# NikolayKrivosheev/Distributed-deep-learning-on-personal-computers

Measured on AMD Instinct MI355X. Metric: images/sec (whole node), U-Net 256x256 6-class tiles, higher is better.
Workload: dtype bf16

## Files before the change

csrc/bindings.cpp:

```cpp
#include <ATen/ATen.h>
#include <c10/core/DeviceGuard.h>
#include <c10/hip/HIPStream.h>
#include <torch/library.h>

#include <cstdlib>
#include <mutex>
#include <string>
#include <unordered_map>
#include <vector>

#include "ops.h"

namespace ddlpc {

namespace {

hipStream_t cur_stream() { return c10::hip::getCurrentHIPStream().stream(); }

#define CHECK_DEV(t) TORCH_CHECK((t).is_cuda(), #t " must be a GPU tensor")
#define CHECK_CONTIG(t) TORCH_CHECK((t).is_contiguous(), #t " must be contiguous")
#define CHECK_BF16(t) TORCH_CHECK((t).scalar_type() == at::kBFloat16, #t " must be bf16")
#define CHECK_F32(t) TORCH_CHECK((t).scalar_type() == at::kFloat, #t " must be fp32")

const bf16_t* bptr(const at::Tensor& t) { return reinterpret_cast<const bf16_t*>(t.data_ptr()); }
// ... 28 lines not shown
    TD = 1;
    TW = W >= 16 ? 16 : 8;
    TH = BM / TW;
  } else {
    TW = W >= 16 ? 16 : 8;
    TH = 4;
    TD = BM / (TW * TH);
  }
}

int pick_bn(int Cout) {
  if (Cout <= 32) return 32;
  if (Cout <= 64) return 64;
  return 128;
}

}

namespace {
thread_local std::string g_last_path;
}
void set_last_path(const std::string& path) { g_last_path = path; }
std::string last_path() { return g_last_path; }

namespace {
const char* const kKnobs[] = {"CROP_LDS_T"};
bool knob_registered(const std::string& name) {
  for (const char* k : kKnobs)
    if (k[0] != 0 && name == k) return true;
  return false;
}
std::mutex g_knob_mu;
std::unordered_map<std::string, int>& knob_map() {
  static std::unordered_map<std::string, int> m;
  return m;
}
}

int knob(const char* name, int def) {
  TORCH_CHECK(knob_registered(name), "knob '", name, "' read but not listed in kKnobs");
  std::lock_guard<std::mutex> lk(g_knob_mu);
  auto& m = knob_map();
  auto it = m.find(name);
  if (it != m.end()) return it->second;
  const std::string env = std::string("DDLPC_") + name;
  const char* e = getenv(env.c_str());
  const int v = e ? atoi(e) : def;
  m.emplace(name, v);
  return v;
// ... 970 lines not shown
                                    const at::Tensor& labels, const at::Tensor& out3,
                                    const c10::optional<at::Tensor>& gscale, int64_t ignore_index,
                                    const c10::optional<at::Tensor>& dw_out,
                                    const c10::optional<at::Tensor>& db_out,
                                    const c10::optional<at::Tensor>& bn4, bool store_da) {
  CHECK_DEV(a); CHECK_CONTIG(a);
  c10::DeviceGuard guard(a.device());
  const int C = (int)a.size(-1), K = (int)Wh.size(0);
  const float* pbn = bn4_ptr(bn4, C);
  TORCH_CHECK(head_supported(C, K), "head kernel: unsupported (C, K)");
  TORCH_CHECK(store_da || pbn != nullptr, "head_ce_bwd: store_da=False needs the deferred BN (bn4)");
  const long long P = a.numel() / C;
  const int nb = head_ce_bwd_blocks(C, K, pbn != nullptr, P, num_cus());
  auto fopts = a.options().dtype(at::kFloat);
  at::Tensor dA = store_da ? at::empty_like(a) : at::empty({0}, a.options());
  at::Tensor part = at::empty({nb, K * C + K}, fopts);
  at::Tensor bnpart = pbn != nullptr ? at::empty({nb, 2, C}, fopts) : at::empty({0}, fopts);
  head_ce_bwd_launch(bptr(a), Wh.data_ptr<float>(), bh.data_ptr<float>(), labels.data_ptr<int64_t>(),
                     fptr_opt(gscale), out3.data_ptr<float>(), 0, store_da ? bptr_mut(dA) : nullptr,
                     part.data_ptr<float>(), nb, P, C, K, (int)ignore_index, pbn,
                     pbn != nullptr ? bnpart.data_ptr<float>() : nullptr, cur_stream());
  set_last_path(std::string("head_ce_bwd:") + head_variant(C) + (pbn != nullptr ? ":defer" : "") +
                (store_da ? "" : ":stats"));
  const bool into = dw_out.has_value() && dw_out->defined();
  at::Tensor sums = reduce_rows(part, nb, K * C + K);
  if (into) {
    TORCH_CHECK(dw_out->is_contiguous() && db_out->is_contiguous(), "grad outs must be contiguous");
    scatter_sums_launch(sums.data_ptr<double>(), K * C, dw_out->data_ptr<float>(), 2, 0, 0, 0, 1.f,
                        true, cur_stream());
    scatter_sums_launch(sums.data_ptr<double>() + K * C, K, db_out->data_ptr<float>(), 2, 0, 0, 0,
                        1.f, true, cur_stream());
    at::Tensor none = at::empty({0}, fopts);
    return {dA, none, none, bnpart};
  }
  at::Tensor red = at::empty({K * C + K}, fopts);
  scatter_sums_launch(sums.data_ptr<double>(), K * C + K, red.data_ptr<float>(), 2, 0, 0, 0, 1.f,
                      false, cur_stream());
  at::Tensor dW = red.narrow(0, 0, K * C).view({K, C});
  at::Tensor db = red.narrow(0, K * C, K);
  return {dA, dW, db, bnpart};
}

std::vector<at::Tensor> head_ce_bn_bwd(const at::Tensor& a, const at::Tensor& Wh, const at::Tensor& bh,
                                       const at::Tensor& labels, const at::Tensor& out3,
                                       const c10::optional<at::Tensor>& gscale, int64_t ignore_index,
                                       const at::Tensor& bn4, const at::Tensor& partial,
// ... 9 lines not shown
    const long long P = a.numel() / C;
    TORCH_CHECK(C == 32 && K <= 16 && P % (groups * 16) == 0,
                "head_ce_bn_bwd groups: C = 32 head, pixels per group a multiple of 16");
    CHECK_F32(bn4); CHECK_CONTIG(bn4); CHECK_F32(partial); CHECK_CONTIG(partial); CHECK_F32(gamma);
    TORCH_CHECK(bn4.numel() == groups * 4 * C && partial.numel() % (groups * 2 * C) == 0,
                "head_ce_bn_bwd groups: bn4 [groups][4][C], partial [groups * R][2][C]");
    auto fopts = a.options().dtype(at::kFloat);
    const bool into = dgamma_out.has_value() && dgamma_out->defined();
    at::Tensor dgamma = into ? *dgamma_out : at::empty({C}, fopts);
    at::Tensor dbeta = into ? *dbeta_out : at::empty({C}, fopts);
    at::Tensor coefs = at::empty({groups, 3, C}, fopts);
    at::Tensor gsum = at::empty({groups, 2, C}, a.options().dtype(at::kDouble));
    const int nb = (int)(partial.numel() / (groups * 2 * C));
    bn_group_grad_rows_launch(partial.data_ptr<float>(), nb, (int)groups, C, (double)(P / groups),
                              gamma.data_ptr<float>(), bn4.data_ptr<float>(), dgamma.data_ptr<float>(),
                              dbeta.data_ptr<float>(), into, coefs.data_ptr<float>(),
                              gsum.data_ptr<double>(), ps, cur_stream());
    at::Tensor dY = at::empty_like(a);
    head_bn_apply_launch(bptr(a), Wh.data_ptr<float>(), bh.data_ptr<float>(), labels.data_ptr<int64_t>(),
                         fptr_opt(gscale), out3.data_ptr<float>(), bn4.data_ptr<float>(),
                         coefs.data_ptr<float>(), bptr_mut(dY), P, C, K, (int)ignore_index, num_cus(),
                         cur_stream(), (int)groups);
    set_last_path("head_ce_bn_bwd:head32:groups");
    return {dY, dgamma, dbeta};
  }
  const float* pbn = bn4_ptr(bn4, C);
  TORCH_CHECK(head_supported(C, K), "head kernel: unsupported (C, K)");
  CHECK_F32(partial); CHECK_CONTIG(partial); CHECK_F32(gamma);
  TORCH_CHECK(partial.numel() % (2 * C) == 0 && partial.numel() > 0, "partial rows must be [R][2][C]");
  const long long P = a.numel() / C;
  const int nb = (int)(partial.numel() / (2 * C));
  auto fopts = a.options().dtype(at::kFloat);
  const bool into = dgamma_out.has_value() && dgamma_out->defined();
  at::Tensor dgamma = into ? *dgamma_out : at::empty({C}, fopts);
  at::Tensor dbeta = into ? *dbeta_out : at::empty({C}, fopts);
  at::Tensor coefs = at::empty({3, C}, fopts);
  const float* s = pbn;
  if (nb <= 2048) {
    bn_grad_finalize_rows_launch(partial.data_ptr<float>(), nb, C, (double)P, gamma.data_ptr<float>(),
                                 s + C, dgamma.data_ptr<float>(), dbeta.data_ptr<float>(),
                                 coefs.data_ptr<float>(), into, cur_stream(), ps);
  } else {
    at::Tensor sums = reduce_rows(partial, nb, 2 * C);
    bn_grad_finalize_launch(sums.data_ptr<double>(), C, (double)P, gamma.data_ptr<float>(), s + C,
                            dgamma.data_ptr<float>(), dbeta.data_ptr<float>(),
                            coefs.data_ptr<float>(), into, cur_stream(), ps);
  }
  at::Tensor dY = at::empty_like(a);
  head_bn_apply_launch(bptr(a), Wh.data_ptr<float>(), bh.data_ptr<float>(), labels.data_ptr<int64_t>(),
                       fptr_opt(gscale), out3.data_ptr<float>(), pbn, coefs.data_ptr<float>(),
                       bptr_mut(dY), P, C, K, (int)ignore_index, num_cus(), cur_stream());
  set_last_path(std::string("head_ce_bn_bwd:") + head_variant(C));
  return {dY, dgamma, dbeta};
}

std::vector<at::Tensor> head_ce_fwd_stats(const at::Tensor& a, const at::Tensor& Wh,
                                          const at::Tensor& bh, const at::Tensor& labels,
                                          int64_t ignore_index, const at::Tensor& bn4,
                                          int64_t groups) {
  CHECK_DEV(a); CHECK_CONTIG(a); CHECK_BF16(a); CHECK_CONTIG(labels);
  TORCH_CHECK(labels.scalar_type() == at::kLong, "labels must be int64");
  c10::DeviceGuard guard(a.device());
  const int C = (int)a.size(-1), K = (int)Wh.size(0);
  const long long P = a.numel() / C;
  const float* pbn = nullptr;
  if (groups > 1) {
    CHECK_F32(bn4); CHECK_CONTIG(bn4);
    TORCH_CHECK(C == 32 && K <= 16 && P % (groups * 16) == 0 && bn4.numel() == groups * 4 * C,
                "head_ce_fwd_stats groups: C = 32 head, bn4 [groups][4][C], pixels per group a "
                "multiple of 16");
    pbn = bn4.data_ptr<float>();
  } else {
    pbn = bn4_ptr(bn4, C);
  }
  TORCH_CHECK(head_supported(C, K), "head kernel: unsupported (C, K)");
  TORCH_CHECK(labels.numel() == P, "labels / activation pixel count mismatch");
  const int nb = head_fwd_stats_blocks(C, K, P, num_cus(), groups > 1 ? (int)groups : 1);
  auto fopts = a.options().dtype(at::kFloat);
  at::Tensor wrows = at::empty({nb, K * C + K}, fopts);
  at::Tensor brows = at::empty({nb, 2, C}, fopts);
  at::Tensor lrows = at::empty({nb, 3}, fopts);
  at::Tensor out3 = at::empty({3}, fopts);
  head_ce_fwd_stats_launch(bptr(a), Wh.data_ptr<float>(), bh.data_ptr<float>(), labels.data_ptr<int64_t>(),
                           pbn, wrows.data_ptr<float>(), brows.data_ptr<float>(), lrows.data_ptr<float>(),
                           out3.data_ptr<float>(), nb, P, C, K, (int)ignore_index, cur_stream(),
                           groups > 1 ? (int)groups : 1);
  set_last_path(std::string("head_ce_fwd_stats:") + head_variant(C) + (groups > 1 ? ":groups" : ""));
  return {out3, wrows, brows};
}

std::vector<at::Tensor> head_wgrad_from_rows(const at::Tensor& rows, const at::Tensor& scale, int64_t K,
                                             int64_t C, const c10::optional<at::Tensor>& dw_out,
                                             const c10::optional<at::Tensor>& db_out) {
  CHECK_F32(rows); CHECK_CONTIG(rows); CHECK_F32(scale);
  c10::DeviceGuard guard(rows.device());
  TORCH_CHECK(rows.dim() == 2 && rows.size(1) == K * C + K, "rows must be [R][K*C + K]");
  const int R = (int)rows.size(0);
  at::Tensor sums = reduce_rows(rows, R, K * C + K);
  auto fopts = rows.options();
  const bool into = dw_out.has_value() && dw_out->defined();
  if (into) {
    TORCH_CHECK(dw_out->is_contiguous() && db_out->is_contiguous(), "grad outs must be contiguous");
    if (db_out->data_ptr<float>() == dw_out->data_ptr<float>() + K * C) {
      scatter_sums_dscale_launch(sums.data_ptr<double>(), K * C + K, dw_out->data_ptr<float>(),
                                 scale.data_ptr<float>(), true, cur_stream());
    } else {
      scatter_sums_dscale_launch(sums.data_ptr<double>(), K * C, dw_out->data_ptr<float>(),
                                 scale.data_ptr<float>(), true, cur_stream());
      scatter_sums_dscale_launch(sums.data_ptr<double>() + K * C, K, db_out->data_ptr<float>(),
                                 scale.data_ptr<float>(), true, cur_stream());
// ... 363 lines not shown
}

int64_t set_cu_reserve(int64_t k) {
  if (k >= 0) g_cu_reserve = (int)std::min<int64_t>(k, std::max(0, phys_cus() - 8));
  return num_cus();
}

void comm_proxy(const at::Tensor& g, int64_t blocks, int64_t passes) {
  CHECK_DEV(g); CHECK_CONTIG(g); CHECK_F32(g);
  TORCH_CHECK(reinterpret_cast<uintptr_t>(g.data_ptr()) % 16 == 0, "comm_proxy: 16-byte aligned buffer");
  c10::DeviceGuard guard(g.device());
  if (g.numel() == 0) return;
  comm_proxy_launch(g.data_ptr<float>(), g.numel(), (int)blocks, (int)passes, cur_stream());
}

}

}

TORCH_LIBRARY(ddlpc, m) {
  m.def("set_cu_reserve(int k) -> int", &ddlpc::set_cu_reserve);
  m.def("set_knob(str name, int value) -> int", &ddlpc::set_knob);
  m.def("last_path() -> str", &ddlpc::last_path);
  m.def("comm_proxy(Tensor(a!) g, int blocks, int passes) -> ()");
  m.def("conv3_fwd(Tensor x1, Tensor? x2, Tensor w, Tensor? bias, Tensor? pscale, Tensor? pshift, "
        "int cout, int co1, bool stats, Tensor? pscale2=None, Tensor? pshift2=None, Tensor? bnb_y=None, "
        "Tensor? bnb_s4=None, int groups=0) -> Tensor[]");
  m.def("conv3_wgrad(Tensor dy, Tensor x1, Tensor? x2, Tensor? pscale, Tensor? pshift, Tensor(a!)? out=None, "
        "Tensor? pscale2=None, Tensor? pshift2=None, Tensor? dy_y=None, Tensor? dy_s4=None, "
        "Tensor? dy_coefs=None, int cin_real=0, int groups=0, Tensor(b!)? dy_out=None) -> Tensor");
  m.def("conv3_bwd32(Tensor dy, Tensor y, Tensor s4, Tensor wd, Tensor(a!)? dw_out=None, int groups=0) -> Tensor[]");
  m.def("reduce_rows(Tensor partial, int R, int N) -> Tensor");
  m.def("bn_finalize(Tensor partial, float count, Tensor gamma, Tensor beta, Tensor(a!) running_mean, "
        "Tensor(b!) running_var, float momentum, float eps, bool update_running, Tensor(c!)? nbt) -> Tensor");
  m.def("bn_relu_apply(Tensor y, Tensor stats4, bool pool, bool full=True) -> Tensor[]");
  m.def("bn_running_apply(Tensor(a!) running_mean, Tensor(b!) running_var, Tensor slots, float momentum, "
        "Tensor(c!)? nbt=None) -> ()");
  m.def("bn_grad_coefs(Tensor partial, Tensor y, Tensor stats4, Tensor gamma, "
        "Tensor(a!)? dgamma_out=None, Tensor(b!)? dbeta_out=None) -> Tensor[]");
  m.def("bn_group_finalize(Tensor y, int groups, Tensor gamma, Tensor beta, float eps, "
        "Tensor(a!)? arena=None, int aoff=0) -> Tensor");
  m.def("bn_group_apply(Tensor y, Tensor stats4, int groups, bool pool) -> Tensor[]");
  m.def("bn_running_apply_all(Tensor entries, Tensor(a!) arena, int K, int maxC, float momentum) -> ()");
  m.def("bn_group_backward(Tensor? dA, Tensor? dP, Tensor y, Tensor stats4, Tensor gamma, int groups, "
        "Tensor(a!)? dgamma_out=None, Tensor(b!)? dbeta_out=None, Tensor? partial=None) -> Tensor[]");
  m.def("bn_group_finalize_rows(Tensor partial, int groups, float count, Tensor gamma, Tensor beta, "
// ... 24 lines not shown
        "float wd, float step_size, float inv_sqrt_bc2) -> ()");
  m.def("adam_step_dev(Tensor(a!) p, Tensor g, Tensor(b!) m, Tensor(c!) v, Tensor(d!) scal, "
        "float lr, float b1, float b2, float eps, float wd) -> ()");
  m.def("weight_pack(Tensor entries, int n, int max_elems) -> ()");
  m.def("codec_absmax(Tensor x, Tensor seg) -> Tensor");
  m.def("codec_encode(Tensor x, Tensor seg, Tensor scales, int codec) -> Tensor");
  m.def("codec_decode_sum(Tensor(a!) out, Tensor q, Tensor scales, Tensor w, Tensor seg, int codec) -> ()");
  m.def("bilinear_up2(Tensor x) -> Tensor");
  m.def("bilinear_up2_bwd(Tensor dy) -> Tensor");
  m.def("to_nhwc_bf16(Tensor x, int cpad=1) -> Tensor");
  m.def("synth_tiles(Tensor idx, int seed, int classes, int in_ch, int tile, int dims, int grid, "
        "float k, Tensor palette, int cpad) -> Tensor[]");
  m.def("tile_gather(Tensor src, Tensor lab, Tensor idx, int cpad) -> Tensor[]");
  m.def("crop_gather(Tensor scenes, Tensor labels, Tensor table, Tensor params, Tensor? color, "
        "int tile, int cpad) -> Tensor[]");
  m.def("crop_params(Tensor idx, Tensor cum, Tensor table, int seed, int tile, int mode, "
        "float gain_jitter, float bias_jitter) -> Tensor[]");
  m.def("window_gather(Tensor scene, Tensor origins, int tile, int cpad) -> Tensor");
  m.def("head_predict_accum(Tensor a, Tensor Wh, Tensor bh, Tensor origins, Tensor win, Tensor(a!) acc, "
        "Tensor? bn4=None) -> ()");
  m.def("scene_finalize(Tensor acc, int K, Tensor? labels=None, int ignore_index=-100) -> Tensor[]");
}

TORCH_LIBRARY_IMPL(ddlpc, CUDA, m) {
  m.impl("conv3_fwd", &ddlpc::conv3_fwd);
  m.impl("conv3_wgrad", &ddlpc::conv3_wgrad);
  m.impl("bn_finalize", &ddlpc::bn_finalize);
  m.impl("reduce_rows", &ddlpc::reduce_rows);
  m.impl("bn_relu_apply", &ddlpc::bn_relu_apply);
  m.impl("bn_running_apply", &ddlpc::bn_running_apply);
  m.impl("bn_grad_coefs", &ddlpc::bn_grad_coefs);
  m.impl("conv3_bwd32", &ddlpc::conv3_bwd32);
  m.impl("bn_backward", &ddlpc::bn_backward);
  m.impl("bn_group_finalize", &ddlpc::bn_group_finalize);
  m.impl("bn_group_apply", &ddlpc::bn_group_apply);
  m.impl("bn_running_apply_all", &ddlpc::bn_running_apply_all);
  m.impl("bn_group_backward", &ddlpc::bn_group_backward);
  m.impl("bn_group_finalize_rows", &ddlpc::bn_group_finalize_rows);
  m.impl("convt_fwd", &ddlpc::convt_fwd);
  m.impl("convt_dgrad", &ddlpc::convt_dgrad);
  m.impl("convt_wgrad", &ddlpc::convt_wgrad);
  m.impl("convt_bwd_fused", &ddlpc::convt_bwd_fused);
  m.impl("head_ce_fwd", &ddlpc::head_ce_fwd);
  m.impl("head_ce_bwd", &ddlpc::head_ce_bwd);
  m.impl("head_ce_bn_bwd", &ddlpc::head_ce_bn_bwd);
  m.impl("head_ce_fwd_stats", &ddlpc::head_ce_fwd_stats);
  m.impl("head_wgrad_from_rows", &ddlpc::head_wgrad_from_rows);
// ... 22 lines not shown
```

csrc/head_ce.hip:

```cpp
#include "common.h"
#include "ops.h"

namespace ddlpc {

namespace {

constexpr int MAXC = 64, MAXK = 16;



template <int C, bool DEFER>
DDLPC_DEVICE void act8(const bf16_t* ap, int c8, const float* sBN, float (&f)[8]) {
  const uint4 v = *reinterpret_cast<const uint4*>(ap + c8);
  unpack8(v, f);
  if (DEFER) {
    const float* vb = sBN + opaque_zero();
#pragma unroll
    for (int j = 0; j < 8; ++j) f[j] = fmaxf(fmaf(f[j], vb[c8 + j], vb[C + c8 + j]), 0.f);
    unpack8(pack8(f), f);
  }
}

template <int C, int KP>
DDLPC_DEVICE void load_head(const float* Wh, const float* bh, int K, float* sW, float* sb) {
// ... 726 lines not shown
      float y8[8], d[4], o8[8], lse, zy;
      int am;
      uint4 pk, fb;
      uint2 bh2, bl2;
      head32_step<true, false>(yv, lab, valid, sW + opaque_zero() + lane, sc, sh, gs, ignore_index, g, y8, fb, d, bh2, bl2, o8, pk,
                               lse, zy, am);
      float rr[8], o[8], is[8], nm[8], k1[8], m1[8], m2[8];
      unpack8(pk, rr);
      k8(2, is); k8(3, nm); k8(4, k1); k8(5, m1); k8(6, m2);
#pragma unroll
      for (int jj = 0; jj < 8; ++jj) {
        const float av2 = fmaf(y8[jj], sc[jj], sh[jj]);
        const float dyh = av2 > 0.f ? rr[jj] : 0.f;
        const float xh = fmaf(y8[jj], is[jj], nm[jj]);
        o[jj] = k1[jj] * (dyh - m1[jj] - xh * m2[jj]);
      }
      if (valid) *reinterpret_cast<uint4*>(dY + px * C + 8 * g) = pack8(o);
      const long long sl = s + HEAD32_DA * wstride;
      load(sl < steps ? sl : s0, q4.y[j], q4.l[j]);
    }
  }
}

template <int C, int K, bool DEFER>
__global__ __launch_bounds__(256) void head_logits_kernel(const bf16_t* __restrict__ a, const float* __restrict__ Wh,
                                   const float* __restrict__ bh, float* __restrict__ out,
                                   long long P, long long HW, const float* __restrict__ bn4,
                                   int Kreal) {
  __shared__ __attribute__((aligned(16))) float sBNm[4 * C];
  __shared__ float sW[K * C], sb[K];
  load_head<C, K>(Wh, bh, Kreal, sW, sb);
  const float* sBN = DEFER ? load_bn<C>(bn4, sBNm, false) : nullptr;
  __syncthreads();
#pragma unroll 1
  for (long long px = blockIdx.x * (long long)blockDim.x + threadIdx.x; px < P;
       px += (long long)gridDim.x * blockDim.x) {
    float z[K];
    logits_of<C, K, DEFER>(a + px * C, sW, sb, sBN, z);
    const long long n = px / HW, s = px % HW;
#pragma unroll
    for (int k = 0; k < K; ++k)
      if (k < Kreal) out[(n * Kreal + k) * HW + s] = z[k];
  }
}

template <int C, int K, bool DEFER>
// ... 68 lines not shown
}

bool head_supported(int C, int K) {
  return HEAD_SWITCH(C, K, (void)0);
}

void head_ce_fwd_launch(const bf16_t* a, const float* Wh, const float* bh, const int64_t* labels,
                        float* partial, float* out3, const float* bn4, int nblocks, long long P,
                        int C, int K, int ignore_index, hipStream_t st) {
  if (bn4 != nullptr)
    HEAD_SWITCH(C, K, hipLaunchKernelGGL((head_ce_fwd_kernel<CC, KK, true>), dim3(nblocks), dim3(256), 0,
                                         st, a, Wh, bh, labels, partial, P, ignore_index, bn4, K));
  else
    HEAD_SWITCH(C, K, hipLaunchKernelGGL((head_ce_fwd_kernel<CC, KK, false>), dim3(nblocks), dim3(256), 0,
                                         st, a, Wh, bh, labels, partial, P, ignore_index, bn4, K));
  hipLaunchKernelGGL(ce_finalize_kernel, dim3(1), dim3(256), 0, st, partial, nblocks, out3);
}

namespace {
int head32_per_cu(const void* fn) {
  int n = 0;
  return hipOccupancyMaxActiveBlocksPerMultiprocessor(&n, fn, 256, 0) == hipSuccess && n > 0 ? n : 1;
}
int head32_grid(long long P, int per_cu, int num_cus) {
  const long long steps4 = ((P + 15) / 16 + 3) / 4;
  return (int)std::max<long long>(1, std::min<long long>(steps4, (long long)per_cu * num_cus));
}
int head32_bwd_per_cu() {
  static int n = std::min({head32_per_cu(reinterpret_cast<const void*>(&head32_kernel<true, true, false>)),
                           head32_per_cu(reinterpret_cast<const void*>(&head32_kernel<true, false, false>)),
                           head32_per_cu(reinterpret_cast<const void*>(&head32_kernel<false, true, false>))});
  return n;
}
}

int head_ce_bwd_blocks(int C, int K, bool , long long P, int num_cus) {
  if (C == 32) return head32_grid(P, head32_bwd_per_cu(), num_cus);
  int per_cu = 8;
  auto occ = [&](const void* fn) {
    int n = 0;
    if (hipOccupancyMaxActiveBlocksPerMultiprocessor(&n, fn, 256, 0) == hipSuccess && n > 0)
      per_cu = std::min(per_cu, n);
    else
      per_cu = std::min(per_cu, 1);
  };
  HEAD_SWITCH(C, K, occ(reinterpret_cast<const void*>(&head_ce_bwd_kernel<CC, KK, true>)));
  HEAD_SWITCH(C, K, occ(reinterpret_cast<const void*>(&head_ce_bwd_kernel<CC, KK, false>)));
  const long long ppb = 256 / (C / 8);
  return (int)std::max<long long>(1, std::min<long long>((P + ppb - 1) / ppb, (long long)per_cu * num_cus));
}

void head_ce_bwd_launch(const bf16_t* a, const float* Wh, const float* bh, const int64_t* labels,
                        const float* gscale, const float* stats3, int , bf16_t* dA,
                        float* dW_partial, int nblocks, long long P, int C, int K,
                        int ignore_index, const float* bn4, float* bnpart, hipStream_t st) {
  if (C == 32 && K <= MAXK) {
    if (bn4 != nullptr && dA == nullptr)
      hipLaunchKernelGGL((head32_kernel<true, false, false>), dim3(nblocks), dim3(256), 0, st, a, Wh, bh,
                         labels, gscale, stats3, dA, dW_partial, P, ignore_index, bn4, bnpart, K, nullptr, 1, 0LL);
    else if (bn4 != nullptr)
      hipLaunchKernelGGL((head32_kernel<true, true, false>), dim3(nblocks), dim3(256), 0, st, a, Wh, bh,
                         labels, gscale, stats3, dA, dW_partial, P, ignore_index, bn4, bnpart, K, nullptr, 1, 0LL);
    else
      hipLaunchKernelGGL((head32_kernel<false, true, false>), dim3(nblocks), dim3(256), 0, st, a, Wh, bh,
                         labels, gscale, stats3, dA, dW_partial, P, ignore_index, bn4, bnpart, K, nullptr, 1, 0LL);
    return;
  }
  if (bn4 != nullptr && dA == nullptr)
    HEAD_SWITCH(C, K, hipLaunchKernelGGL((head_ce_bwd_kernel<CC, KK, true, false>), dim3(nblocks), dim3(256), 0,
                                         st, a, Wh, bh, labels, gscale, stats3, dA, dW_partial, P,
                                         ignore_index, bn4, bnpart, K));
  else if (bn4 != nullptr)
    HEAD_SWITCH(C, K, hipLaunchKernelGGL((head_ce_bwd_kernel<CC, KK, true>), dim3(nblocks), dim3(256), 0,
                                         st, a, Wh, bh, labels, gscale, stats3, dA, dW_partial, P,
                                         ignore_index, bn4, bnpart, K));
  else
    HEAD_SWITCH(C, K, hipLaunchKernelGGL((head_ce_bwd_kernel<CC, KK, false>), dim3(nblocks), dim3(256), 0,
                                         st, a, Wh, bh, labels, gscale, stats3, dA, dW_partial, P,
                                         ignore_index, bn4, bnpart, K));
}

int head_fwd_stats_blocks(int C, int K, long long P, int num_cus, int groups) {
  if (C == 32 && K <= MAXK) {
    static const int n = head32_per_cu(reinterpret_cast<const void*>(&head32_kernel<true, false, true>));
    const int nb = head32_grid(P, n, num_cus);
    return groups > 1 ? groups * std::max(1, nb / groups) : nb;
  }
  return head_ce_bwd_blocks(C, K, true, P, num_cus);
}

void head_ce_fwd_stats_launch(const bf16_t* a, const float* Wh, const float* bh,
                              const int64_t* labels, const float* bn4, float* dW_partial,
                              float* bnpart, float* loss_partial, float* out3, int nblocks,
                              long long P, int C, int K, int ignore_index, hipStream_t st, int groups) {
  if (C == 32 && K <= MAXK)
    hipLaunchKernelGGL((head32_kernel<true, false, true>), dim3(nblocks), dim3(256), 0, st, a, Wh, bh, labels,
                       nullptr, nullptr, nullptr, dW_partial, P, ignore_index, bn4, bnpart, K, loss_partial,
                       groups, groups > 1 ? P / groups / 16 : 0LL);
  else
    HEAD_SWITCH(C, K, hipLaunchKernelGGL((head_ce_bwd_kernel<CC, KK, true, false, true>), dim3(nblocks),
                                         dim3(256), 0, st, a, Wh, bh, labels, nullptr, nullptr, nullptr,
                                         dW_partial, P, ignore_index, bn4, bnpart, K, loss_partial));
  hipLaunchKernelGGL(ce_finalize_kernel, dim3(1), dim3(256), 0, st, loss_partial, nblocks, out3);
}

int head_bn_apply_blocks(long long P, int C) {
  const long long ppb = 256 / (C / 8);
  const int cap = 4096;
  return (int)std::max<long long>(1, std::min<long long>((P + 2 * ppb - 1) / (2 * ppb), cap));
}

void head_bn_apply_launch(const bf16_t* a, const float* Wh, const float* bh, const int64_t* labels,
                          const float* gscale, const float* stats3, const float* bn4,
                          const float* coefs, bf16_t* dY, long long P, int C, int K,
                          int ignore_index, int num_cus, hipStream_t st, int groups) {
  if (C == 32 && K <= MAXK) {
    static const int per_cu = head32_per_cu(reinterpret_cast<const void*>(&head32_apply_kernel));
    const int nb = head32_grid(P, per_cu, num_cus);
    const int grid = groups > 1 ? groups * std::max(1, nb / groups) : nb;
    hipLaunchKernelGGL(head32_apply_kernel, dim3(grid), dim3(256), 0, st, a, Wh, bh,
                       labels, gscale, stats3, bn4, coefs, dY, P, ignore_index, K, groups,
                       groups > 1 ? P / groups / 16 : 0LL);
    return;
  }
  const int nb = head_bn_apply_blocks(P, C);
  HEAD_SWITCH(C, K, hipLaunchKernelGGL((head_bn_apply_kernel<CC, KK>), dim3(nb), dim3(256), 0, st,
                                       a, Wh, bh, labels, gscale, stats3, bn4, coefs, dY, P,
                                       ignore_index, K));
}

void head_logits_launch(const bf16_t* a, const float* Wh, const float* bh, float* logits,
                        long long P, long long HW, int C, int K, const float* bn4, hipStream_t st) {
  const int grid = (int)std::min<long long>((P + 255) / 256, 4096);
  if (bn4 != nullptr)
    HEAD_SWITCH(C, K, hipLaunchKernelGGL((head_logits_kernel<CC, KK, true>), dim3(grid), dim3(256), 0, st,
                                         a, Wh, bh, logits, P, HW, bn4, K));
  else
    HEAD_SWITCH(C, K, hipLaunchKernelGGL((head_logits_kernel<CC, KK, false>), dim3(grid), dim3(256), 0, st,
// ... 18 lines not shown
```

csrc/ops.h:

```cpp
#pragma once

#include <hip/hip_runtime.h>
#include <stdint.h>

#include <algorithm>
#include <string>

#include "common.h"

namespace ddlpc {

struct ConvFwdArgs {
  int dims;
  int N, D, H, W;
  int C1, C2, Cin, CinW;
  int Cout, Co1;
  int taps;
  const bf16_t* X1;
  const bf16_t* X2;
  const float* pscale;
  const float* pshift;
  const float* pscale2;
  const float* pshift2;
  const bf16_t* Wt;
// ... 125 lines not shown
                         int D, int H, int W, int C, hipStream_t st);
int bn_bwd_reduce_blocks(long long pixels_or_quads);
bool bn_group_supported(int dims, bool pool, int D, int H, int W, int C);
int bn_group_stats_rows(long long gpix, int C, int groups);
void bn_group_stats_finalize_launch(const bf16_t* y, int groups, long long gpix, int C,
                                    const float* gamma, const float* beta, float eps, float* out4,
                                    float* arena, long long astride, float* partial_scratch,
                                    int nb, hipStream_t st);
int bn_group_bwd_rows(long long items_per_group, int groups);
void bn_group_backward_launch(const bf16_t* dA, const bf16_t* dP, const bf16_t* y,
                              const float* stats4, const float* gamma, float* dgamma, float* dbeta,
                              bool accumulate, float* coefs, float* partial_scratch, int nb,
                              bf16_t* dY, int dims, int groups, int N, int D, int H, int W, int C,
                              hipStream_t st, bool have_partial, double* gsum_scratch);
void bn_group_grad_rows_launch(const float* partial, int nb, int groups, int C, double count,
                               const float* gamma, const float* stats4, float* dgamma, float* dbeta,
                               bool accumulate, float* coefs, double* gsum_scratch,
                               const float* dscale, hipStream_t st);
void bn_group_finalize_rows_launch(const float* partial, int nb, int groups, long long gpix, int C,
                                   const float* gamma, const float* beta, float eps, float* out4,
                                   float* arena, long long astride, hipStream_t st);

bool head_supported(int C, int K);
void head_ce_fwd_launch(const bf16_t* a, const float* Wh, const float* bh, const int64_t* labels,
                        float* partial, float* out3, const float* bn4, int nblocks, long long P,
                        int C, int K, int ignore_index, hipStream_t st);
int head_ce_bwd_blocks(int C, int K, bool defer, long long P, int num_cus);
int head_fwd_stats_blocks(int C, int K, long long P, int num_cus, int groups = 1);
void head_ce_bwd_launch(const bf16_t* a, const float* Wh, const float* bh, const int64_t* labels,
                        const float* gscale, const float* stats3, int unused, bf16_t* dA,
                        float* dW_partial, int nblocks, long long P, int C, int K,
                        int ignore_index, const float* bn4, float* bnpart, hipStream_t st);
void head_ce_fwd_stats_launch(const bf16_t* a, const float* Wh, const float* bh,
                              const int64_t* labels, const float* bn4, float* dW_partial,
                              float* bnpart, float* loss_partial, float* out3, int nblocks,
                              long long P, int C, int K, int ignore_index, hipStream_t st,
                              int groups = 1);
void head_bn_apply_launch(const bf16_t* a, const float* Wh, const float* bh, const int64_t* labels,
                          const float* gscale, const float* stats3, const float* bn4,
                          const float* coefs, bf16_t* dY, long long P, int C, int K,
                          int ignore_index, int num_cus, hipStream_t st, int groups = 1);
void head_logits_launch(const bf16_t* a, const float* Wh, const float* bh, float* logits_nchw,
                        long long P, long long HW, int C, int K, const float* bn4, hipStream_t st);
void head_predict_accum_launch(const bf16_t* a, const float* Wh, const float* bh, const int* origins,
                               const float* win, float* acc, int B, int tile, int H, int W, int KA,
                               int C, int K, const float* bn4, hipStream_t st);
// ... 65 lines not shown

void synth_tiles_launch(const int64_t* idx, int B, uint32_t seed, int classes, int in_ch, int tile,
                        int dims, int grid, float k, const float* palette, int cpad, bf16_t* x,
                        int64_t* y, hipStream_t st);
void tile_gather_launch(const uint8_t* src, const uint8_t* lab, const int64_t* idx, int B,
                        long long S, int in_ch, int cpad, long long N, bf16_t* x, int64_t* y,
                        hipStream_t st);
void crop_params_launch(const int64_t* idx, int B, const int64_t* cum, const int64_t* table, int n,
                        uint32_t seed, int tile, int mode, float gain_jitter, float bias_jitter,
                        int* params, float* color, hipStream_t st);
int crop_gather_blocks(int tile);
void crop_gather_launch(const uint8_t* src, const uint8_t* lab, const int64_t* table, int n,
                        long long total_px, const int* params, const float* color, int B, int in_ch,
                        int tile, int cpad, bool lds_transpose, bf16_t* x, int64_t* y, hipStream_t st);

void bn_running_apply_launch(float* rm, float* rv, const float* slots, int K, int C, long long stride,
                             float momentum, int64_t* nbt, hipStream_t st);
void bn_running_apply_all_launch(const int64_t* entries, int L, int maxC, const float* arena, int K,
                                 long long stride, float momentum, hipStream_t st);

int knob(const char* name, int def);

void set_last_path(const std::string& path);

void comm_proxy_launch(float* g, long long n, int blocks, int passes, hipStream_t st);

}
```

Baseline: 7760.

## Add paired 32-pixel MFMA head kernels for C=32 segmentation head

Adds new head32p kernels for forward-stats, backward and BN-apply of the 32-channel CE head. Each wave step now handles 32 pixels: the two 16-pixel halves run through 16x16x32 MFMAs and are combined with permlane16_swap reductions, with software-pipelined loads two or three steps deep. The goal is to raise per-instruction work and cut per-step overhead in this memory-bound head. A HEAD32_PAIR knob (on by default) selects the path, and a last_variant debug hook reports which variant ran. The cost is much more complex lane mapping, which needs permlane16_swap support.

```diff
diff --git a/csrc/bindings.cpp b/csrc/bindings.cpp
--- a/csrc/bindings.cpp
+++ b/csrc/bindings.cpp
@@ -74,9 +74,14 @@
 }
 void set_last_path(const std::string& path) { g_last_path = path; }
 std::string last_path() { return g_last_path; }
-
 namespace {
-const char* const kKnobs[] = {"CROP_LDS_T"};
+thread_local std::string g_last_variant;
+}
+void set_last_variant(const std::string& variant) { g_last_variant = variant; }
+std::string last_variant() { return g_last_variant; }
+
+namespace {
+const char* const kKnobs[] = {"CROP_LDS_T", "HEAD32_PAIR"};
 bool knob_registered(const std::string& name) {
   for (const char* k : kKnobs)
     if (k[0] != 0 && name == k) return true;
@@ -1093,6 +1098,7 @@
                      pbn != nullptr ? bnpart.data_ptr<float>() : nullptr, cur_stream());
   set_last_path(std::string("head_ce_bwd:") + head_variant(C) + (pbn != nullptr ? ":defer" : "") +
                 (store_da ? "" : ":stats"));
+  set_last_variant(head32_paired(C, K, 1) ? "pair" : "single");
   const bool into = dw_out.has_value() && dw_out->defined();
   at::Tensor sums = reduce_rows(part, nb, K * C + K);
   if (into) {
@@ -1148,6 +1154,7 @@
                          coefs.data_ptr<float>(), bptr_mut(dY), P, C, K, (int)ignore_index, num_cus(),
                          cur_stream(), (int)groups);
     set_last_path("head_ce_bn_bwd:head32:groups");
+    set_last_variant("single");
     return {dY, dgamma, dbeta};
   }
   const float* pbn = bn4_ptr(bn4, C);
@@ -1177,6 +1184,7 @@
                        fptr_opt(gscale), out3.data_ptr<float>(), pbn, coefs.data_ptr<float>(),
                        bptr_mut(dY), P, C, K, (int)ignore_index, num_cus(), cur_stream());
   set_last_path(std::string("head_ce_bn_bwd:") + head_variant(C));
+  set_last_variant(head32_paired(C, K, 1) ? "pair" : "single");
   return {dY, dgamma, dbeta};
 }
 
@@ -1212,6 +1220,7 @@
                            out3.data_ptr<float>(), nb, P, C, K, (int)ignore_index, cur_stream(),
                            groups > 1 ? (int)groups : 1);
   set_last_path(std::string("head_ce_fwd_stats:") + head_variant(C) + (groups > 1 ? ":groups" : ""));
+  set_last_variant(head32_paired(C, K, (int)groups) ? "pair" : "single");
   return {out3, wrows, brows};
 }
 
@@ -1621,6 +1630,7 @@
   m.def("set_cu_reserve(int k) -> int", &ddlpc::set_cu_reserve);
   m.def("set_knob(str name, int value) -> int", &ddlpc::set_knob);
   m.def("last_path() -> str", &ddlpc::last_path);
+  m.def("last_variant() -> str", &ddlpc::last_variant);
   m.def("comm_proxy(Tensor(a!) g, int blocks, int passes) -> ()");
   m.def("conv3_fwd(Tensor x1, Tensor? x2, Tensor w, Tensor? bias, Tensor? pscale, Tensor? pshift, "
         "int cout, int co1, bool stats, Tensor? pscale2=None, Tensor? pshift2=None, Tensor? bnb_y=None, "
@@ -1691,7 +1701,12 @@
   m.def("scene_finalize(Tensor acc, int K, Tensor? labels=None, int ignore_index=-100) -> Tensor[]");
 }
 
+TORCH_LIBRARY_IMPL(ddlpc, CPU, m) {
+  m.impl("last_variant", &ddlpc::last_variant);
+}
+
 TORCH_LIBRARY_IMPL(ddlpc, CUDA, m) {
+  m.impl("last_variant", &ddlpc::last_variant);
   m.impl("conv3_fwd", &ddlpc::conv3_fwd);
   m.impl("conv3_wgrad", &ddlpc::conv3_wgrad);
   m.impl("bn_finalize", &ddlpc::bn_finalize);
diff --git a/csrc/head_ce.hip b/csrc/head_ce.hip
--- a/csrc/head_ce.hip
+++ b/csrc/head_ce.hip
@@ -772,6 +772,440 @@
   }
 }
 
+
+DDLPC_DEVICE float rows2_sum(float v) {
+  auto a = __builtin_amdgcn_permlane16_swap(__builtin_bit_cast(unsigned, v), __builtin_bit_cast(unsigned, v),
+                                            false, false);
+  return __builtin_bit_cast(float, (unsigned)a[0]) + __builtin_bit_cast(float, (unsigned)a[1]);
+}
+DDLPC_DEVICE float rows2_max(float v) {
+  auto a = __builtin_amdgcn_permlane16_swap(__builtin_bit_cast(unsigned, v), __builtin_bit_cast(unsigned, v),
+                                            false, false);
+  return fmaxf(__builtin_bit_cast(float, (unsigned)a[0]), __builtin_bit_cast(float, (unsigned)a[1]));
+}
+DDLPC_DEVICE int rows2_min_i(int v) {
+  auto a = __builtin_amdgcn_permlane16_swap((unsigned)v, (unsigned)v, false, false);
+  return min((int)a[0], (int)a[1]);
+}
+
+struct Head32PW { uint4 zh[2], zl[2]; uint2 th[2][2], tl[2][2]; f32x4_t b4; };
+DDLPC_DEVICE Head32PW head32p_weights(const float* __restrict__ Wh, const float* __restrict__ bh, int Kreal,
+                                      int lane) {
+  const int n = lane & 15, g = lane >> 4;
+  Head32PW w;
+#pragma unroll
+  for (int s = 0; s < 2; ++s) {
+    float hi[8], lo[8];
+#pragma unroll
+    for (int j = 0; j < 8; ++j) {
+      const float v = ((n >> 3) == s && (n & 7) < Kreal) ? Wh[(n & 7) * 32 + 8 * g + j] : 0.f;
+      hi[j] = lo_bf(pack2(v, 0.f));
+      lo[j] = v - hi[j];
+    }
+    w.zh[s] = pack8(hi);
+    w.zl[s] = pack8(lo);
+#pragma unroll
+    for (int t = 0; t < 2; ++t) {
+      const int ch = 8 * (n >> 2) + 4 * t + (n & 3);
+      float h4[4], l4[4];
+#pragma unroll
+      for (int i = 0; i < 4; ++i) {
+        const int k = 4 * (g & 1) + i;
+        const float v = ((g >> 1) == s && k < Kreal) ? Wh[k * 32 + ch] : 0.f;
+        h4[i] = lo_bf(pack2(v, 0.f));
+        l4[i] = v - h4[i];
+      }
+      w.th[s][t] = make_uint2(pack2(h4[0], h4[1]), pack2(h4[2], h4[3]));
+      w.tl[s][t] = make_uint2(pack2(l4[0], l4[1]), pack2(l4[2], l4[3]));
+    }
+  }
+#pragma unroll
+  for (int i = 0; i < 4; ++i) w.b4[i] = 4 * (g & 1) + i < Kreal ? bh[4 * (g & 1) + i] : -INFINITY;
+  return w;
+}
+
+template <bool DEFER>
+DDLPC_DEVICE uint4 head32p_act(const uint4 yv, const float (&y8)[8], const float (&sc)[8], const float (&sh)[8]) {
+  if (!DEFER) return yv;
+  uint32_t o[4];
+#pragma unroll
+  for (int j = 0; j < 4; ++j) {
+    const f32x2_t r2 = __builtin_elementwise_fma(f32x2_t{y8[2 * j], y8[2 * j + 1]},
+                                                 f32x2_t{sc[2 * j], sc[2 * j + 1]},
+                                                 f32x2_t{sh[2 * j], sh[2 * j + 1]});
+    const uint32_t pb = __builtin_bit_cast(uint32_t, __builtin_convertvector(r2, bf16x2_t));
+    o[j] = __builtin_bit_cast(uint32_t, __builtin_elementwise_max(__builtin_bit_cast(i16x2_t, pb),
+                                                                  i16x2_t{0, 0}));
+  }
+  return make_uint4(o[0], o[1], o[2], o[3]);
+}
+
+template <bool LOSS>
+DDLPC_DEVICE void head32p_softmax(const uint4 fzA, const uint4 fzB, const int lab, const bool vown,
+                                  const Head32PW* __restrict__ wl, float gs, int ignore_index, int g,
+                                  float (&d)[4], uint2& bh2, uint2& bl2, float& lse, float& zy, int& am) {
+  f32x4_t z = mfma16x16x32(wl->zh[0], fzA, wl->b4);
+  z = mfma16x16x32(wl->zl[0], fzA, z);
+  z = mfma16x16x32(wl->zh[1], fzB, z);
+  z = mfma16x16x32(wl->zl[1], fzB, z);
+  const int c0 = 4 * (g & 1);
+  float m = fmaxf(fmaxf(z[0], z[1]), fmaxf(z[2], z[3]));
+  m = rows2_max(m);
+  float e[4], se = 0.f;
+#pragma unroll
+  for (int i = 0; i < 4; ++i) { e[i] = __expf(z[i] - m); se += e[i]; }
+  se = rows2_sum(se);
+  const float inv = __builtin_amdgcn_rcpf(se);
+  const bool live = vown && lab != ignore_index;
+  bool hot[4];
+#pragma unroll
+  for (int i = 0; i < 4; ++i) {
+    hot[i] = c0 + i == lab;
+    d[i] = live ? (e[i] * inv - (hot[i] ? 1.f : 0.f)) * gs : 0.f;
+  }
+  if (LOSS) {
+    lse = m + __logf(se);
+    float t = 0.f;
+    int c = 16;
+#pragma unroll
+    for (int i = 0; i < 4; ++i) {
+      t = hot[i] ? z[i] : t;
+      c = (z[i] == m && c == 16) ? c0 + i : c;
+    }
+    zy = rows2_sum(t);
+    am = rows2_min_i(c);
+  }
+  const uint32_t h01 = pack2(d[0], d[1]), h23 = pack2(d[2], d[3]);
+  const float dl0 = d[0] - lo_bf(h01), dl1 = d[1] - hi_bf(h01);
+  const float dl2 = d[2] - lo_bf(h23), dl3 = d[3] - hi_bf(h23);
+  bh2 = make_uint2(h01, h23);
+  bl2 = make_uint2(pack2(dl0, dl1), pack2(dl2, dl3));
+}
+
+DDLPC_DEVICE void head32p_da(const Head32PW* __restrict__ wl, const int s, const uint2 bh2, const uint2 bl2,
+                             float (&o8)[8], uint4& pk) {
+#pragma unroll
+  for (int t = 0; t < 2; ++t) {
+    f32x4_t o = f32x4_t{0.f, 0.f, 0.f, 0.f};
+    const uint2 th = wl->th[s][t], tl = wl->tl[s][t];
+    o = mfma16x16x16(th, bh2, o);
+    o = mfma16x16x16(th, bl2, o);
+    o = mfma16x16x16(tl, bh2, o);
+#pragma unroll
+    for (int i = 0; i < 4; ++i) o8[4 * t + i] = o[i];
+  }
+  pk = pack8(o8);
+}
+
+constexpr int HEAD32P_D = 2;
+constexpr int HEAD32P_DA = 3;
+
+template <int D>
+struct Head32PLd {
+  uint4 y[D][2];
+  int l[D];
+};
+
+template <bool DEFER, bool LOSS>
+DDLPC_DEVICE void head32p_reduce(char (*sT)[4096], float (*sred)[4][24], const int wave, const f32x4_t (&dw)[2],
+                                 const float (&db)[4], const float (&b1)[8], const float (&b2)[8],
+                                 const float (&ls)[3], float* __restrict__ dWp, float* __restrict__ bnpart,
+                                 float* __restrict__ lossp, const int Kreal);
+
+template <bool DEFER, bool STORE, bool LOSS>
+__global__ __launch_bounds__(256, 4) void head32p_kernel(
+    const bf16_t* __restrict__ a, const float* __restrict__ Wh, const float* __restrict__ bh,
+    const int64_t* __restrict__ labels, const float* __restrict__ gscale,
+    const float* __restrict__ stats3, bf16_t* __restrict__ dA, float* __restrict__ dWp,
+    long long P, int ignore_index, const float* __restrict__ bn4, float* __restrict__ bnpart,
+    int Kreal, float* __restrict__ lossp) {
+  static_assert(!LOSS || (DEFER && !STORE), "the fused forward is the deferred stats pass");
+  constexpr int C = 32;
+  __shared__ __attribute__((aligned(16))) char sT[4][4096];
+  __shared__ float sred[4][4][24];
+  __shared__ __attribute__((aligned(16))) float sK[4][C];
+  __shared__ Head32PW sW[64];
+  const int tid = threadIdx.x, lane = tid & 63, wave = __builtin_amdgcn_readfirstlane(tid >> 6);
+  const int n = lane & 15, g = lane >> 4;
+  if (tid < 64) sW[tid] = head32p_weights(Wh, bh, Kreal, lane);
+  if (DEFER && tid < C) {
+    sK[0][tid] = bn4[2 * C + tid];
+    sK[1][tid] = bn4[3 * C + tid];
+    sK[2][tid] = bn4[C + tid];
+    sK[3][tid] = -bn4[tid] * bn4[C + tid];
+  }
+  char* tA = sT[wave];
+  char* tDh = tA + 2048;
+  char* tDl = tA + 3072;
+  *reinterpret_cast<uint4*>(tDh + lane * 32) = make_uint4(0, 0, 0, 0);
+  *reinterpret_cast<uint4*>(tDh + lane * 32 + 16) = make_uint4(0, 0, 0, 0);
+  __syncthreads();
+  const float cnt = LOSS ? 1.f : stats3[2];
+  const float gs = LOSS ? 1.f : (gscale != nullptr ? gscale[0] : 1.0f) / (cnt > 0.f ? cnt : 1.f);
+  const int q = (lane & 15) >> 2, pq = lane & 3;
+  const int rA = (8 * g + q) * 64 + pq * 8;
+  const int rD = (8 * g + q) * 32 + pq * 8;
+  const int wD = (n + 16 * (g >> 1)) * 32 + g * 8;
+  f32x4_t dw[2] = {f32x4_t{0.f, 0.f, 0.f, 0.f}, f32x4_t{0.f, 0.f, 0.f, 0.f}};
+  float db[4] = {0.f, 0.f, 0.f, 0.f}, b1[8], b2[8], ls[3] = {0.f, 0.f, 0.f};
+#pragma unroll
+  for (int j = 0; j < 8; ++j) { b1[j] = 0.f; b2[j] = 0.f; }
+  const long long steps = (P + 31) / 32;
+  const long long wstride = (long long)gridDim.x * 4;
+  const long long s0 = (long long)blockIdx.x * 4 + wave;
+  auto load = [&](long long st, uint4 (&yv)[2], int& lb) __attribute__((always_inline)) {
+    const long long pa = st * 32 + n, pb = pa + 16;
+    const long long ca = pa < P ? pa : 0, cb = pb < P ? pb : 0;
+    yv[0] = *reinterpret_cast<const uint4*>(a + ca * C + 8 * g);
+    yv[1] = *reinterpret_cast<const uint4*>(a + cb * C + 8 * g);
+    lb = reinterpret_cast<const int*>(labels)[2 * (g < 2 ? ca : cb)];
+  };
+  Head32PLd<HEAD32P_D> q4;
+#pragma unroll
+  for (int j = 0; j < HEAD32P_D; ++j) load(s0 + j * wstride < steps ? s0 + j * wstride : s0, q4.y[j], q4.l[j]);
+#pragma unroll 1
+  for (long long sb = s0; sb < steps; sb += HEAD32P_D * wstride) {
+#pragma unroll
+    for (int j = 0; j < HEAD32P_D; ++j) {
+      const long long s = sb + j * wstride;
+      const int lab = q4.l[j];
+      const long long px = s * 32 + n;
+      const bool vs[2] = {s < steps && px < P, s < steps && px + 16 < P};
+      const bool vown = g < 2 ? vs[0] : vs[1];
+      float sc[8], sh[8];
+      if (DEFER) {
+        const float4* kp = reinterpret_cast<const float4*>(&sK[0][0] + opaque_zero() + 8 * g);
+        const float4 a0 = kp[0], a1 = kp[1], c0 = kp[8], c1 = kp[9];
+        sc[0] = a0.x; sc[1] = a0.y; sc[2] = a0.z; sc[3] = a0.w; sc[4] = a1.x; sc[5] = a1.y; sc[6] = a1.z; sc[7] = a1.w;
+        sh[0] = c0.x; sh[1] = c0.y; sh[2] = c0.z; sh[3] = c0.w; sh[4] = c1.x; sh[5] = c1.y; sh[6] = c1.z; sh[7] = c1.w;
+      } else {
+#pragma unroll
+        for (int jj = 0; jj < 8; ++jj) { sc[jj] = 0.f; sh[jj] = 0.f; }
+      }
+      const Head32PW* wl = sW + opaque_zero() + lane;
+      uint4 fz[2];
+#pragma unroll
+      for (int t = 0; t < 2; ++t) {
+        float y8[8];
+        unpack8(q4.y[j][t], y8);
+        const uint4 fb = head32p_act<DEFER>(q4.y[j][t], y8, sc, sh);
+        fz[t] = vs[t] ? fb : make_uint4(0, 0, 0, 0);
+        *reinterpret_cast<uint4*>(tA + (16 * t + n) * 64 + g * 16) = fz[t];
+      }
+      float d[4], lse = 0.f, zy = 0.f;
+      int am = 0;
+      uint2 bh2, bl2;
+      head32p_softmax<LOSS>(fz[0], fz[1], lab, vown, wl, gs, ignore_index, g, d, bh2, bl2, lse, zy, am);
+      *reinterpret_cast<uint2*>(tDh + wD) = bh2;
+      *reinterpret_cast<uint2*>(tDl + wD) = bl2;
+      {
+        const uint2 h0 = lds_read_tr16(tDh + rD), h1 = lds_read_tr16(tDh + rD + 128);
+        const uint2 l0 = lds_read_tr16(tDl + rD), l1 = lds_read_tr16(tDl + rD + 128);
+        const uint4 ah = make_uint4(h0.x, h0.y, h1.x, h1.y), al = make_uint4(l0.x, l0.y, l1.x, l1.y);
+#pragma unroll
+        for (int nt = 0; nt < 2; ++nt) {
+          const uint2 b0 = lds_read_tr16(tA + rA + nt * 32), b1r = lds_read_tr16(tA + rA + nt * 32 + 256);
+          const uint4 b = make_uint4(b0.x, b0.y, b1r.x, b1r.y);
+          dw[nt] = mfma16x16x32(ah, b, dw[nt]);
+          dw[nt] = mfma16x16x32(al, b, dw[nt]);
+        }
+      }
+#pragma unroll
+      for (int i = 0; i < 4; ++i) db[i] += d[i];
+      if (LOSS) {
+        const bool cnt_px = (g & 1) == 0 && vown;
+        const bool lv = cnt_px && lab != ignore_index;
+        ls[0] += lv ? lse - zy : 0.f;
+        ls[2] += lv ? 1.f : 0.f;
+        ls[1] += (cnt_px && am == lab) ? 1.f : 0.f;
+      }
+#pragma unroll
+      for (int t = 0; t < 2; ++t) {
+        float o8[8];
+        uint4 pk;
+        head32p_da(wl, t, bh2, bl2, o8, pk);
+        if (STORE && vs[t]) *reinterpret_cast<uint4*>(dA + (px + 16 * t) * C + 8 * g) = pk;
+        if (DEFER) {
+          float y8[8], r[8];
+          unpack8(q4.y[j][t], y8);
+          if (LOSS) {
+#pragma unroll
+            for (int jj = 0; jj < 8; ++jj) r[jj] = o8[jj];
+          } else {
+            unpack8(pk, r);
+          }
+          const float4* kp = reinterpret_cast<const float4*>(&sK[2][0] + opaque_zero() + 8 * g);
+          const float4 a0 = kp[0], a1 = kp[1], c0 = kp[8], c1 = kp[9];
+          const float xi[8] = {a0.x, a0.y, a0.z, a0.w, a1.x, a1.y, a1.z, a1.w};
+          const float xm[8] = {c0.x, c0.y, c0.z, c0.w, c1.x, c1.y, c1.z, c1.w};
+          const bool valid = vs[t];
+#pragma unroll
+          for (int jj = 0; jj < 8; jj += 2) {
+            const f32x2_t y2 = {y8[jj], y8[jj + 1]};
+            const f32x2_t a2 = __builtin_elementwise_fma(y2, f32x2_t{sc[jj], sc[jj + 1]},
+                                                         f32x2_t{sh[jj], sh[jj + 1]});
+            const f32x2_t x2 = __builtin_elementwise_fma(y2, f32x2_t{xi[jj], xi[jj + 1]},
+                                                         f32x2_t{xm[jj], xm[jj + 1]});
+            const f32x2_t d2 = {(valid && a2.x > 0.f) ? r[jj] : 0.f, (valid && a2.y > 0.f) ? r[jj + 1] : 0.f};
+            f32x2_t s1 = {b1[jj], b1[jj + 1]}, s2 = {b2[jj], b2[jj + 1]};
+            s1 += d2;
+            s2 = __builtin_elementwise_fma(d2, x2, s2);
+            b1[jj] = s1.x; b1[jj + 1] = s1.y; b2[jj] = s2.x; b2[jj + 1] = s2.y;
+          }
+        }
+      }
+      const long long sl = s + HEAD32P_D * wstride;
+      load(sl < steps ? sl : s0, q4.y[j], q4.l[j]);
+    }
+  }
+  head32p_reduce<DEFER, LOSS>(sT, sred, wave, dw, db, b1, b2, ls, dWp, bnpart, lossp, Kreal);
+}
+
+DDLPC_DEVICE int lane_id_again() {
+  int l;
+  asm volatile("v_mbcnt_lo_u32_b32 %0, -1, 0\n\tv_mbcnt_hi_u32_b32 %0, -1, %0" : "=v"(l));
+  return l;
+}
+
+template <bool DEFER, bool LOSS>
+DDLPC_DEVICE void head32p_reduce(char (*sT)[4096], float (*sred)[4][24], const int wave, const f32x4_t (&dw)[2],
+                                 const float (&db)[4], const float (&b1)[8], const float (&b2)[8],
+                                 const float (&ls)[3], float* __restrict__ dWp, float* __restrict__ bnpart,
+                                 float* __restrict__ lossp, const int Kreal) {
+  constexpr int C = 32;
+  const int lane = lane_id_again(), tid = wave * 64 + lane;
+  const int n = lane & 15, g = lane >> 4;
+  float* wd = reinterpret_cast<float*>(sT[wave]);
+#pragma unroll
+  for (int nt = 0; nt < 2; ++nt)
+#pragma unroll
+    for (int i = 0; i < 4; ++i) wd[(4 * g + i) * 32 + nt * 16 + n] = dw[nt][i];
+  float red[23];
+#pragma unroll
+  for (int i = 0; i < 4; ++i) red[i] = row16_sum(db[i]);
+#pragma unroll
+  for (int j = 0; j < 8; ++j) { red[4 + j] = DEFER ? row16_sum(b1[j]) : 0.f; red[12 + j] = DEFER ? row16_sum(b2[j]) : 0.f; }
+#pragma unroll
+  for (int i = 0; i < 3; ++i) red[20 + i] = LOSS ? row16_sum(ls[i]) : 0.f;
+  if (n == 0)
+#pragma unroll
+    for (int i = 0; i < 23; ++i) sred[wave][g][i] = red[i];
+  __syncthreads();
+  const int nout = Kreal * C + Kreal;
+  for (int o = tid; o < nout; o += 256) {
+    float t = 0.f;
+    if (o < Kreal * C) {
+      const int k = o / C, c = o % C;
+      for (int wv = 0; wv < 4; ++wv) {
+        const float* w32 = reinterpret_cast<const float*>(sT[wv]);
+        t += w32[k * 32 + c] + w32[(k + 8) * 32 + c];
+      }
+    } else {
+      const int k = o - Kreal * C;
+      for (int wv = 0; wv < 4; ++wv) t += sred[wv][k >> 2][k & 3] + sred[wv][2 + (k >> 2)][k & 3];
+    }
+    dWp[(long long)blockIdx.x * nout + o] = t;
+  }
+  if (DEFER)
+    for (int o = tid; o < 2 * C; o += 256) {
+      const int half = o / C, c = o % C;
+      float t = 0.f;
+      for (int wv = 0; wv < 4; ++wv) t += sred[wv][c >> 3][4 + 8 * half + (c & 7)];
+      bnpart[(long long)blockIdx.x * 2 * C + o] = t;
+    }
+  if (LOSS && tid < 3) {
+    float t = 0.f;
+    for (int wv = 0; wv < 4; ++wv) t += sred[wv][0][20 + tid] + sred[wv][2][20 + tid];
+    lossp[(long long)blockIdx.x * 3 + tid] = t;
+  }
+}
+
+__global__ __launch_bounds__(256, 4) void head32p_apply_kernel(
+    const bf16_t* __restrict__ a, const float* __restrict__ Wh, const float* __restrict__ bh,
+    const int64_t* __restrict__ labels, const float* __restrict__ gscale,
+    const float* __restrict__ stats3, const float* __restrict__ bn4,
+    const float* __restrict__ coefs, bf16_t* __restrict__ dY, long long P, int ignore_index,
+    int Kreal) {
+  constexpr int C = 32;
+  __shared__ __attribute__((aligned(16))) float sK[7][C];
+  __shared__ Head32PW sW[64];
+  const int tid = threadIdx.x, lane = tid & 63, wave = __builtin_amdgcn_readfirstlane(tid >> 6);
+  const int n = lane & 15, g = lane >> 4;
+  if (tid < 64) sW[tid] = head32p_weights(Wh, bh, Kreal, lane);
+  if (tid < C) {
+    sK[0][tid] = bn4[2 * C + tid]; sK[1][tid] = bn4[3 * C + tid];
+    sK[2][tid] = bn4[C + tid]; sK[3][tid] = -bn4[tid] * bn4[C + tid];
+    sK[4][tid] = coefs[tid]; sK[5][tid] = coefs[C + tid]; sK[6][tid] = coefs[2 * C + tid];
+  }
+  __syncthreads();
+  const float cnt = stats3[2];
+  const float gs = (gscale != nullptr ? gscale[0] : 1.0f) / (cnt > 0.f ? cnt : 1.f);
+  const long long steps = (P + 31) / 32;
+  const long long wstride = (long long)gridDim.x * 4;
+  const long long s0 = (long long)blockIdx.x * 4 + wave;
+  auto load = [&](long long st, uint4 (&yv)[2], int& lb) __attribute__((always_inline)) {
+    const long long pa = st * 32 + n, pb = pa + 16;
+    const long long ca = pa < P ? pa : 0, cb = pb < P ? pb : 0;
+    yv[0] = *reinterpret_cast<const uint4*>(a + ca * C + 8 * g);
+    yv[1] = *reinterpret_cast<const uint4*>(a + cb * C + 8 * g);
+    lb = reinterpret_cast<const int*>(labels)[2 * (g < 2 ? ca : cb)];
+  };
+  auto k8 = [&](int r, float (&v)[8]) __attribute__((always_inline)) {
+    const float4* kp = reinterpret_cast<const float4*>(&sK[r][0] + opaque_zero() + 8 * g);
+    const float4 a0 = kp[0], a1 = kp[1];
+    v[0] = a0.x; v[1] = a0.y; v[2] = a0.z; v[3] = a0.w; v[4] = a1.x; v[5] = a1.y; v[6] = a1.z; v[7] = a1.w;
+  };
+  Head32PLd<HEAD32P_DA> q4;
+#pragma unroll
+  for (int j = 0; j < HEAD32P_DA; ++j) load(s0 + j * wstride < steps ? s0 + j * wstride : s0, q4.y[j], q4.l[j]);
+#pragma unroll 1
+  for (long long sb = s0; sb < steps; sb += HEAD32P_DA * wstride) {
+#pragma unroll
+    for (int j = 0; j < HEAD32P_DA; ++j) {
+      const long long s = sb + j * wstride;
+      const int lab = q4.l[j];
+      const long long px = s * 32 + n;
+      const bool vs[2] = {s < steps && px < P, s < steps && px + 16 < P};
+      const bool vown = g < 2 ? vs[0] : vs[1];
+      float sc[8], sh[8];
+      k8(0, sc);
+      k8(1, sh);
+      const Head32PW* wl = sW + opaque_zero() + lane;
+      uint4 fz[2];
+#pragma unroll
+      for (int t = 0; t < 2; ++t) {
+        float y8[8];
+        unpack8(q4.y[j][t], y8);
+        const uint4 fb = head32p_act<true>(q4.y[j][t], y8, sc, sh);
+        fz[t] = vs[t] ? fb : make_uint4(0, 0, 0, 0);
+      }
+      float d[4], lse, zy;
+      int am;
+      uint2 bh2, bl2;
+      head32p_softmax<false>(fz[0], fz[1], lab, vown, wl, gs, ignore_index, g, d, bh2, bl2, lse, zy, am);
+#pragma unroll
+      for (int t = 0; t < 2; ++t) {
+        float o8[8], y8[8], rr[8], o[8], is[8], nm[8], k1[8], m1[8], m2[8];
+        uint4 pk;
+        head32p_da(wl, t, bh2, bl2, o8, pk);
+        unpack8(q4.y[j][t], y8);
+        unpack8(pk, rr);
+        k8(2, is); k8(3, nm); k8(4, k1); k8(5, m1); k8(6, m2);
+#pragma unroll
+        for (int jj = 0; jj < 8; ++jj) {
+          const float av2 = fmaf(y8[jj], sc[jj], sh[jj]);
+          const float dyh = av2 > 0.f ? rr[jj] : 0.f;
+          const float xh = fmaf(y8[jj], is[jj], nm[jj]);
+          o[jj] = k1[jj] * (dyh - m1[jj] - xh * m2[jj]);
+        }
+        if (vs[t]) *reinterpret_cast<uint4*>(dY + (px + 16 * t) * C + 8 * g) = pack8(o);
+      }
+      const long long sl = s + HEAD32P_DA * wstride;
+      load(sl < steps ? sl : s0, q4.y[j], q4.l[j]);
+    }
+  }
+}
+
 template <int C, int K, bool DEFER>
 __global__ __launch_bounds__(256) void head_logits_kernel(const bf16_t* __restrict__ a, const float* __restrict__ Wh,
                                    const float* __restrict__ bh, float* __restrict__ out,
@@ -886,8 +1320,8 @@
   int n = 0;
   return hipOccupancyMaxActiveBlocksPerMultiprocessor(&n, fn, 256, 0) == hipSuccess && n > 0 ? n : 1;
 }
-int head32_grid(long long P, int per_cu, int num_cus) {
-  const long long steps4 = ((P + 15) / 16 + 3) / 4;
+int head32_grid(long long P, int per_cu, int num_cus, int step_px = 16) {
+  const long long steps4 = ((P + step_px - 1) / step_px + 3) / 4;
   return (int)std::max<long long>(1, std::min<long long>(steps4, (long long)per_cu * num_cus));
 }
 int head32_bwd_per_cu() {
@@ -896,9 +1330,20 @@
                            head32_per_cu(reinterpret_cast<const void*>(&head32_kernel<false, true, false>))});
   return n;
 }
+int head32p_bwd_per_cu() {
+  static int n = std::min({head32_per_cu(reinterpret_cast<const void*>(&head32p_kernel<true, true, false>)),
+                           head32_per_cu(reinterpret_cast<const void*>(&head32p_kernel<true, false, false>)),
+                           head32_per_cu(reinterpret_cast<const void*>(&head32p_kernel<false, true, false>))});
+  return n;
+}
+}
+
+bool head32_paired(int C, int K, int groups) {
+  return C == 32 && K <= 8 && groups <= 1 && knob("HEAD32_PAIR", 1) != 0;
 }
 
 int head_ce_bwd_blocks(int C, int K, bool , long long P, int num_cus) {
+  if (head32_paired(C, K, 1)) return head32_grid(P, head32p_bwd_per_cu(), num_cus, 32);
   if (C == 32) return head32_grid(P, head32_bwd_per_cu(), num_cus);
   int per_cu = 8;
   auto occ = [&](const void* fn) {
@@ -918,6 +1363,18 @@
                         const float* gscale, const float* stats3, int , bf16_t* dA,
                         float* dW_partial, int nblocks, long long P, int C, int K,
                         int ignore_index, const float* bn4, float* bnpart, hipStream_t st) {
+  if (head32_paired(C, K, 1)) {
+    if (bn4 != nullptr && dA == nullptr)
+      hipLaunchKernelGGL((head32p_kernel<true, false, false>), dim3(nblocks), dim3(256), 0, st, a, Wh, bh,
+                         labels, gscale, stats3, dA, dW_partial, P, ignore_index, bn4, bnpart, K, nullptr);
+    else if (bn4 != nullptr)
+      hipLaunchKernelGGL((head32p_kernel<true, true, false>), dim3(nblocks), dim3(256), 0, st, a, Wh, bh,
+                         labels, gscale, stats3, dA, dW_partial, P, ignore_index, bn4, bnpart, K, nullptr);
+    else
+      hipLaunchKernelGGL((head32p_kernel<false, true, false>), dim3(nblocks), dim3(256), 0, st, a, Wh, bh,
+                         labels, gscale, stats3, dA, dW_partial, P, ignore_index, bn4, bnpart, K, nullptr);
+    return;
+  }
   if (C == 32 && K <= MAXK) {
     if (bn4 != nullptr && dA == nullptr)
       hipLaunchKernelGGL((head32_kernel<true, false, false>), dim3(nblocks), dim3(256), 0, st, a, Wh, bh,
@@ -945,6 +1402,10 @@
 }
 
 int head_fwd_stats_blocks(int C, int K, long long P, int num_cus, int groups) {
+  if (head32_paired(C, K, groups)) {
+    static const int n = head32_per_cu(reinterpret_cast<const void*>(&head32p_kernel<true, false, true>));
+    return head32_grid(P, n, num_cus, 32);
+  }
   if (C == 32 && K <= MAXK) {
     static const int n = head32_per_cu(reinterpret_cast<const void*>(&head32_kernel<true, false, true>));
     const int nb = head32_grid(P, n, num_cus);
@@ -957,7 +1418,10 @@
                               const int64_t* labels, const float* bn4, float* dW_partial,
                               float* bnpart, float* loss_partial, float* out3, int nblocks,
                               long long P, int C, int K, int ignore_index, hipStream_t st, int groups) {
-  if (C == 32 && K <= MAXK)
+  if (head32_paired(C, K, groups))
+    hipLaunchKernelGGL((head32p_kernel<true, false, true>), dim3(nblocks), dim3(256), 0, st, a, Wh, bh, labels,
+                       nullptr, nullptr, nullptr, dW_partial, P, ignore_index, bn4, bnpart, K, loss_partial);
+  else if (C == 32 && K <= MAXK)
     hipLaunchKernelGGL((head32_kernel<true, false, true>), dim3(nblocks), dim3(256), 0, st, a, Wh, bh, labels,
                        nullptr, nullptr, nullptr, dW_partial, P, ignore_index, bn4, bnpart, K, loss_partial,
                        groups, groups > 1 ? P / groups / 16 : 0LL);
@@ -978,6 +1442,12 @@
                           const float* gscale, const float* stats3, const float* bn4,
                           const float* coefs, bf16_t* dY, long long P, int C, int K,
                           int ignore_index, int num_cus, hipStream_t st, int groups) {
+  if (head32_paired(C, K, groups)) {
+    static const int per_cu = head32_per_cu(reinterpret_cast<const void*>(&head32p_apply_kernel));
+    hipLaunchKernelGGL(head32p_apply_kernel, dim3(head32_grid(P, per_cu, num_cus, 32)), dim3(256), 0, st, a, Wh,
+                       bh, labels, gscale, stats3, bn4, coefs, dY, P, ignore_index, K);
+    return;
+  }
   if (C == 32 && K <= MAXK) {
     static const int per_cu = head32_per_cu(reinterpret_cast<const void*>(&head32_apply_kernel));
     const int nb = head32_grid(P, per_cu, num_cus);
diff --git a/csrc/ops.h b/csrc/ops.h
--- a/csrc/ops.h
+++ b/csrc/ops.h
@@ -171,6 +171,7 @@
                                    float* arena, long long astride, hipStream_t st);
 
 bool head_supported(int C, int K);
+bool head32_paired(int C, int K, int groups);
 void head_ce_fwd_launch(const bf16_t* a, const float* Wh, const float* bh, const int64_t* labels,
                         float* partial, float* out3, const float* bn4, int nblocks, long long P,
                         int C, int K, int ignore_index, hipStream_t st);
@@ -282,6 +283,7 @@
 int knob(const char* name, int def);
 
 void set_last_path(const std::string& path);
+void set_last_variant(const std::string& variant);
 
 void comm_proxy_launch(float* g, long long n, int blocks, int passes, hipStream_t st);
 
```

Result: no change. 7780, median of 6 (+0.2%).
